# locuslab/lcp-physics

Hardware: NVIDIA H100
Metric: LCP solves/sec (LCPFunction fwd+bwd, batch=4096 x 64 contacts, fp32) (higher is better)
Workload: dtype f32 I/O and iterates; the condensed n x n KKT matrix is formed, factored and solved in f64

## Files before the change

lcp_physics_b200/csrc/lcp_cond_kernels.cu:

```cuda
#include "lcp_cond_launch.h"

namespace lcpb200 {
namespace cnd {

template <>
cudaError_t launch_cond_forward_t<LCP_T, LCP_NS>(const CFwdArgs<LCP_T>& a, int grid, cudaStream_t st) {
  if (a.prof) cond_forward_kernel<LCP_T, LCP_NS, true><<<grid, NT, a.P.smem_bytes, st>>>(a);
  else cond_forward_kernel<LCP_T, LCP_NS, false><<<grid, NT, a.P.smem_bytes, st>>>(a);
  return cudaGetLastError();
}

template <>
cudaError_t launch_cond_backward_t<LCP_T, LCP_NS>(const CBwdArgs<LCP_T>& a, int grid, cudaStream_t st) {
  if (a.prof) cond_backward_kernel<LCP_T, LCP_NS, true><<<grid, NT, a.P.smem_bytes, st>>>(a);
  else cond_backward_kernel<LCP_T, LCP_NS, false><<<grid, NT, a.P.smem_bytes, st>>>(a);
  return cudaGetLastError();
}

template <>
cudaError_t launch_cond_jvp_t<LCP_T, LCP_NS>(const CJvpArgs<LCP_T>& a, int grid, cudaStream_t st) {
  const bool dense = a.soa.mass == nullptr;
  if (a.prof) {
    if (dense) cond_jvp_kernel<LCP_T, LCP_NS, true, true><<<grid, NT, a.P.smem_bytes, st>>>(a);
    else cond_jvp_kernel<LCP_T, LCP_NS, true, false><<<grid, NT, a.P.smem_bytes, st>>>(a);
// ... 2 lines not shown
    else cond_jvp_kernel<LCP_T, LCP_NS, false, false><<<grid, NT, a.P.smem_bytes, st>>>(a);
  }
  return cudaGetLastError();
}

template <>
cudaError_t configure_cond_t<LCP_T, LCP_NS>(int smem_bytes, int dyn_max, int* occ) {
  cudaError_t e;
  const void* fns[4] = {(const void*)cond_forward_kernel<LCP_T, LCP_NS, false>, (const void*)cond_backward_kernel<LCP_T, LCP_NS, false>,
                        (const void*)cond_forward_kernel<LCP_T, LCP_NS, true>, (const void*)cond_backward_kernel<LCP_T, LCP_NS, true>};
  for (const void* f : fns)
    if ((e = cudaFuncSetAttribute(f, cudaFuncAttributeMaxDynamicSharedMemorySize, dyn_max)) != cudaSuccess) return e;
  const void* jvp[4] = {(const void*)cond_jvp_kernel<LCP_T, LCP_NS, false, false>, (const void*)cond_jvp_kernel<LCP_T, LCP_NS, true, false>,
                        (const void*)cond_jvp_kernel<LCP_T, LCP_NS, false, true>, (const void*)cond_jvp_kernel<LCP_T, LCP_NS, true, true>};
  for (const void* f : jvp)
    if ((e = cudaFuncSetAttribute(f, cudaFuncAttributeMaxDynamicSharedMemorySize, dyn_max)) != cudaSuccess) return e;
  int of = 0, ob = 0;
  if ((e = cudaOccupancyMaxActiveBlocksPerMultiprocessor(&of, fns[0], NT, smem_bytes)) != cudaSuccess) return e;
  if ((e = cudaOccupancyMaxActiveBlocksPerMultiprocessor(&ob, fns[1], NT, smem_bytes)) != cudaSuccess) return e;
  *occ = of < ob ? of : ob;
  return cudaSuccess;
}

}
}
```

lcp_physics_b200/csrc/lcp_cond_launch.h:

```cpp
#pragma once
#include <cuda_runtime.h>
#include "lcp_condensed.cuh"

namespace lcpb200 {
namespace cnd {

template <typename T, int NS> cudaError_t launch_cond_forward_t(const CFwdArgs<T>& a, int grid, cudaStream_t st);
template <typename T, int NS> cudaError_t launch_cond_backward_t(const CBwdArgs<T>& a, int grid, cudaStream_t st);
template <typename T, int NS> cudaError_t launch_cond_jvp_t(const CJvpArgs<T>& a, int grid, cudaStream_t st);
template <typename T, int NS> cudaError_t configure_cond_t(int smem_bytes, int dyn_max, int* occ);

}
}
```

lcp_physics_b200/csrc/lcp_condensed.cuh:

```cuda
#pragma once
#include "lcp_device.cuh"

namespace lcpb200 {
namespace cnd {

constexpr int NT = 256;
constexpr int UC = 8;
constexpr int CSMAX = 6;
constexpr int KS = 8;
constexpr int LMAX = 16;
constexpr int LU_BW = 2;
constexpr int MISC_BAND_LU = 4;
constexpr int CFLAG_DENSE_LU = 4;
constexpr int STATUS_UNSUPPORTED = -100;

struct CPlan {
  int ok;
  int n, m, e, N, NP, NS;
  int pcap;
  int wcap;
  int smem_bytes;
  int ctas_per_sm;
  int flags;
  int sbytes;
  int o_K, o_W, o_scr, o_bx, o_rdiag, o_Fd, o_Gd, o_As, o_x, o_rx, o_dx, o_qd, o_y, o_ry, o_dy,
      o_s, o_z, o_d, o_rz, o_ds, o_dz, o_rs2, o_red, o_rows, o_posof, o_clist, o_ccols, o_ncols, o_clcnt, o_misc;
};

__host__ __device__ inline size_t al16(size_t x) { return (x + 15) & ~(size_t)15; }
__host__ __device__ inline size_t scratch_bytes(int n, int m, int tsize) {
  return al16((size_t)2 * KS * m * 2) + al16((size_t)2 * KS * m * tsize) + al16((size_t)5 * m * 4) +
         al16((size_t)CSMAX * m * 2) + al16((size_t)8 * m * 4) + al16((size_t)LMAX * n * 2) + al16((size_t)n * 4) + 64;
}

inline size_t carve_plan(CPlan& P, int tsize) {
  size_t o = 0;
  const int n = P.n, m = P.m, e = P.e, NP = P.NP, pcap = P.pcap, wcap = P.wcap;
#define CND_TAKE(field, bytes) do { P.field = (int)o; o += al16((size_t)(bytes)); } while (0)
  size_t kb = (size_t)NP * NP * 8;
  if (scratch_bytes(n, m, tsize) > kb) kb = scratch_bytes(n, m, tsize);
  if ((size_t)8 * NP * 8 > kb) kb = (size_t)8 * NP * 8;
  { const size_t qn = (NP + 31) / 32, sl = (size_t)(NP / qn) * qn * qn * 32 * 8; if (sl > kb) kb = sl; }
  CND_TAKE(o_K, kb);
  CND_TAKE(o_W, (size_t)wcap * 8);
  CND_TAKE(o_scr, (size_t)pcap * 8);
  CND_TAKE(o_bx, (size_t)NP * 8);
  CND_TAKE(o_rdiag, (size_t)NP * 8);
  CND_TAKE(o_Fd, (size_t)wcap * tsize);
  CND_TAKE(o_Gd, (size_t)UC * pcap * tsize);
  CND_TAKE(o_As, (size_t)e * n * tsize);
  CND_TAKE(o_x, n * tsize); CND_TAKE(o_rx, n * tsize); CND_TAKE(o_dx, n * tsize); CND_TAKE(o_qd, n * tsize);
  CND_TAKE(o_y, e * tsize); CND_TAKE(o_ry, e * tsize); CND_TAKE(o_dy, e * tsize);
  CND_TAKE(o_s, m * tsize); CND_TAKE(o_z, m * tsize); CND_TAKE(o_d, m * tsize); CND_TAKE(o_rz, m * tsize);
  CND_TAKE(o_ds, m * tsize); CND_TAKE(o_dz, m * tsize); CND_TAKE(o_rs2, m * tsize);
  CND_TAKE(o_red, 192 * tsize);
  CND_TAKE(o_rows, pcap * 2);
  CND_TAKE(o_posof, m * 2);
  CND_TAKE(o_clist, LMAX * n * 2);
  CND_TAKE(o_ccols, UC * pcap);
  CND_TAKE(o_ncols, pcap);
  CND_TAKE(o_clcnt, n);
  CND_TAKE(o_misc, 16 * 4);
#undef CND_TAKE
  P.sbytes = 16 + (P.o_x - P.o_Fd) + (P.o_y - P.o_qd) + (P.o_misc - P.o_rows);
  return o;
}

extern __shared__ __align__(16) unsigned char cnd_smem[];

template <typename T>
struct CSmem {
  const CPlan& P;
  __device__ __forceinline__ explicit CSmem(const CPlan& p) : P(p) {}
#define CND_ACC(name, type) __device__ __forceinline__ type* name() const { return reinterpret_cast<type*>(cnd_smem + P.o_##name); }
  CND_ACC(K, double) CND_ACC(W, double) CND_ACC(scr, double) CND_ACC(bx, double) CND_ACC(rdiag, double)
  CND_ACC(Fd, T) CND_ACC(Gd, T) CND_ACC(As, T)
  CND_ACC(x, T) CND_ACC(rx, T) CND_ACC(dx, T) CND_ACC(qd, T) CND_ACC(y, T) CND_ACC(ry, T) CND_ACC(dy, T)
  CND_ACC(s, T) CND_ACC(z, T) CND_ACC(d, T) CND_ACC(rz, T) CND_ACC(ds, T) CND_ACC(dz, T) CND_ACC(rs2, T)
  CND_ACC(red, T)
  CND_ACC(rows, unsigned short) CND_ACC(posof, unsigned short) CND_ACC(clist, unsigned short)
  CND_ACC(ccols, unsigned char) CND_ACC(ncols, unsigned char) CND_ACC(clcnt, unsigned char)
  CND_ACC(misc, int)
#undef CND_ACC
};

struct Struct {
  int ncomp, cs;
  int sh;
  int m;
// ... 73 lines not shown
        const unsigned mask = __ballot_sync(FULL, nz);
        const int pos = c + __popc(mask & ((1u << lane) - 1u));
        if (nz && pos < KS) { vals[pos * rows + r] = v[q]; idx[pos * rows + r] = (unsigned short)(j0 + q * 32 + lane); }
        c += __popc(mask);
      }
    }
    if (c > KS) bad = 1;
    if (lane == 0) cnt[r] = c;
  }
  return bad;
}

__device__ __forceinline__ void prefetch_l2(const void* p, size_t bytes) {
  const char* c = reinterpret_cast<const char*>(p);
  for (size_t o = (size_t)threadIdx.x * 128; o < bytes; o += (size_t)NT * 128)
    asm volatile("prefetch.global.L2 [%0];" ::"l"(c + o));
}

template <typename T>
__device__ __noinline__ bool build_structure(const CPlan& P, CSmem<T>& S, Struct& st, const T* __restrict__ Q,
                                             const T* __restrict__ G, const T* __restrict__ A,
                                             const T* __restrict__ F, int* singular) {
  const int n = P.n, m = P.m, e = P.e, tid = threadIdx.x, lane = tid & 31, warp = tid >> 5, pcap = P.pcap;
  prefetch_l2(F, (size_t)m * m * sizeof(T));
  prefetch_l2(G, (size_t)m * n * sizeof(T));
  prefetch_l2(Q, (size_t)n * n * sizeof(T));
  char* sb = reinterpret_cast<char*>(S.K());
  unsigned short* Fi = reinterpret_cast<unsigned short*>(sb);
  unsigned short* Gi = Fi + (size_t)KS * m;
  size_t o = al16((size_t)2 * KS * m * 2);
  T* Fv = reinterpret_cast<T*>(sb + o);
  T* Gv = Fv + (size_t)KS * m;
  o += al16((size_t)2 * KS * m * sizeof(T));
  int* Fcnt = reinterpret_cast<int*>(sb + o);
  int* Gcnt = Fcnt + m;
  int* label = Gcnt + m;
  int* cidx = label + m;
  int* memcnt = cidx + m;
  o += al16((size_t)5 * m * 4);
  unsigned short* memb = reinterpret_cast<unsigned short*>(sb + o);
  o += al16((size_t)CSMAX * m * 2);
  unsigned* cmap = reinterpret_cast<unsigned*>(sb + o);
  o += al16((size_t)8 * m * 4);
  unsigned short* cl_tmp = reinterpret_cast<unsigned short*>(sb + o);
  o += al16((size_t)LMAX * n * 2);
  int* cl_cnt = reinterpret_cast<int*>(sb + o);
  int* flags = S.misc();

  if (tid < 16) flags[tid] = 0;
// ... 729 lines not shown
  const T NEG_INF = -INFINITY, POS_INF = INFINITY;
  T mx[2] = {NEG_INF, NEG_INF};
  T mn[2] = {POS_INF, POS_INF};
  T any[2] = {T(0), T(0)};
  for (int i = threadIdx.x; i < m; i += NT) {
    const T az = -z[i] / dz[i], as = -s[i] / ds[i];
    mx[0] = nan_max(mx[0], az);
    mx[1] = nan_max(mx[1], as);
    if (dz[i] > T(0)) any[0] = T(1); else mn[0] = nan_min(mn[0], az);
    if (ds[i] > T(0)) any[1] = T(1); else mn[1] = nan_min(mn[1], as);
  }
  T v[6] = {mx[0], mx[1], -mn[0], -mn[1], any[0], any[1]};
  block_reduce<T, 6>(v, OpMax(), NEG_INF, red);
  const T fz = (v[0] > T(1)) ? v[0] : T(1);
  const T fs = (v[1] > T(1)) ? v[1] : T(1);
  step_z = (v[4] > T(0)) ? nan_min(-v[2], fz) : -v[2];
  step_s = (v[5] > T(0)) ? nan_min(-v[3], fs) : -v[3];
}

template <typename T>
struct CFwdArgs {
  CPlan P;
  int B;
  const T *Q, *p, *G, *h, *A, *b, *F;
  T *zhat, *nu, *lam, *slack, *resid;
  int *status, *iters;
  T eps;
  int not_improved_lim, max_iter;
  long long* prof;
  EngineSoA<T> soa;
  unsigned char* ssave;
};

template <typename T>
struct CBwdArgs {
  CPlan P;
  int B;
  int R, chunks;
  const T *Q, *G, *A, *F;
  const T *zhat, *nu, *lam, *slack, *g;
  T *dQ, *dp, *dG, *dh, *dA, *db, *dF;
  int* done;
  const int* only;
  unsigned flags;
  const unsigned char* sload;
  EngineSoA<T> soa;
  T *dmass, *dinertia, *dv, *dfext, *dnormal, *dp1, *dp2, *dmu, *drest;
  long long* prof;
};

__device__ __forceinline__ void copy16(unsigned char* dst, const unsigned char* src, int bytes) {
  const uint4* s4 = reinterpret_cast<const uint4*>(src);
  uint4* d4 = reinterpret_cast<uint4*>(dst);
  for (int i = threadIdx.x; i < (bytes >> 4); i += NT) d4[i] = s4[i];
}

__device__ __forceinline__ void save_structure(const CPlan& P, const Struct& st, bool ok, unsigned char* dst) {
  if (threadIdx.x == 0) *reinterpret_cast<int4*>(dst) = make_int4(ok ? st.ncomp : -1, st.cs, st.sh, st.m);
  if (!ok) return;
  const int c1 = P.o_x - P.o_Fd, c2 = P.o_y - P.o_qd, c3 = P.o_misc - P.o_rows;
  copy16(dst + 16, cnd_smem + P.o_Fd, c1);
  copy16(dst + 16 + c1, cnd_smem + P.o_qd, c2);
  copy16(dst + 16 + c1 + c2, cnd_smem + P.o_rows, c3);
}

__device__ __forceinline__ bool load_structure(const CPlan& P, Struct& st, const unsigned char* src) {
  const int4 hd = *reinterpret_cast<const int4*>(src);
  st.ncomp = hd.x; st.cs = hd.y; st.sh = hd.z; st.m = hd.w;
  if (hd.x < 0) return false;
  const int c1 = P.o_x - P.o_Fd, c2 = P.o_y - P.o_qd, c3 = P.o_misc - P.o_rows;
  copy16(cnd_smem + P.o_Fd, src + 16, c1);
  copy16(cnd_smem + P.o_qd, src + 16 + c1, c2);
  copy16(cnd_smem + P.o_rows, src + 16 + c1 + c2, c3);
  return true;
}

template <typename T>
struct SzResid { T sz, resid; };

template <typename T, int CS>
__device__ __noinline__ SzResid<T> fwd_residuals(const CFwdArgs<T>& a, CSmem<T> S, Struct st, int sc) {
  const int nc_ = st.ncomp;
  const CPlan& P = a.P;
  const int n = P.n, m = st.m, e = P.e, tid = threadIdx.x, pcap = P.pcap;
  const T* p = a.p + (size_t)sc * n;
  const T* h = a.h + (size_t)sc * P.m;
  const T* b = e > 0 ? a.b + (size_t)sc * e : nullptr;
  for (int c = tid; c < n; c += NT) {
    T acc = 0;
    const int cnt = S.clcnt()[c];
    for (int l = 0; l < cnt; ++l) {
      const int cp = S.clist()[l * n + c], cc = cp >> 3, pp = cp & 7;
#pragma unroll
      for (int r = 0; r < CS; ++r) {
        const int i = S.rows()[r * nc_ + cc];
        if (i != 0xFFFF) acc = fma(S.Gd()[(size_t)pp * pcap + r * nc_ + cc], S.z()[i], acc);
      }
// ... 138 lines not shown
    pf.lap(CPH_STEP);
    solve_kkt<T, CS, NS>(P, S, st, pf, nullptr, S.rs2(), nullptr, nullptr, S.rx(), S.rz(), S.rs2(), S.ry());
    fwd_step<T>(P, S, m);
    pf.lap(CPH_STEP);
    pf.count(CPH_FACTORS);
    pf.count(CPH_SOLVES, 2);
  }
  if (threadIdx.x == 0) { a.status[sc] = status; a.iters[sc] = it; if (a.resid) a.resid[sc] = best; }
}

template <typename T, int NS, bool PROF>
__global__ void __launch_bounds__(NT, (NS <= 6) ? 2 : 1) cond_forward_kernel(const __grid_constant__ CFwdArgs<T> a) {
  const CPlan& P = a.P;
  CSmem<T> S(P);
  const int n = P.n, m = P.m, e = P.e, tid = threadIdx.x;
  __shared__ int singular_s;
  const T NANV = nan("");
  Prof<PROF> pf(PROF ? a.prof + (size_t)blockIdx.x * CPH_COUNT : nullptr);
  for (int sc = blockIdx.x; sc < a.B; sc += gridDim.x) {
    if (tid == 0) singular_s = 0;
    __syncthreads();
    pf.start();
    Struct st;
    const bool ok = a.soa.mass
        ? build_structure_soa<T>(P, S, st, a.soa, sc, e > 0 ? a.A + (size_t)sc * e * n : nullptr, &singular_s)
        : build_structure<T>(P, S, st, a.Q + (size_t)sc * n * n, a.G + (size_t)sc * m * n,
                             e > 0 ? a.A + (size_t)sc * e * n : nullptr, a.F + (size_t)sc * m * m, &singular_s);
    __syncthreads();
    if (a.ssave) save_structure(P, st, ok, a.ssave + (size_t)sc * P.sbytes);
    pf.lap(CPH_STRUCT);
    if (!ok) {
      if (singular_s) {
        for (int i = tid; i < n; i += NT) a.zhat[(size_t)sc * n + i] = NANV;
        for (int i = tid; i < m; i += NT) { a.lam[(size_t)sc * m + i] = NANV; a.slack[(size_t)sc * m + i] = NANV; }
        for (int i = tid; i < e; i += NT) a.nu[(size_t)sc * e + i] = NANV;
        if (tid == 0) { a.status[sc] = -1; a.iters[sc] = 0; if (a.resid) a.resid[sc] = NANV; }
      } else if (tid == 0) {
        a.status[sc] = STATUS_UNSUPPORTED;
        a.iters[sc] = 0;
      }
      __syncthreads();
      continue;
    }
    if constexpr (LU_BW < NS - 1) mark_band_lu<T>(P, S, st);
    switch (st.cs) {
      case 1: forward_scene<T, NS, 1>(a, S, st, pf, sc); break;
      case 2: forward_scene<T, NS, 2>(a, S, st, pf, sc); break;
      case 3: forward_scene<T, NS, 3>(a, S, st, pf, sc); break;
      case 4: forward_scene<T, NS, 4>(a, S, st, pf, sc); break;
      case 5: forward_scene<T, NS, 5>(a, S, st, pf, sc); break;
      default: forward_scene<T, NS, 6>(a, S, st, pf, sc); break;
    }
    __syncthreads();
  }
}
// ... 481 lines not shown
```

lcp_physics_b200/csrc/lcpb200.cu:

```cuda
#include <cuda_runtime.h>
#include <stdio.h>
#include <string.h>
#include <algorithm>
#include <cfloat>
#include <climits>
#include <cmath>
#include <new>
#include <string>
#include <type_traits>
#include <vector>

#include "../../include/lcpb200.h"
#include "lcp_assemble.cuh"
#include "lcp_launch.h"
#include "lcp_cond_launch.h"
#include "lcp_band_launch.h"
#include "lcp_contacts.cuh"
#include "lcp_ray_launch.h"

using namespace lcpb200;
using cnd::CPlan;

static thread_local std::string g_err;
static int fail(const std::string& s) { g_err = s; return 1; }
// ... 18 lines not shown
};

struct DevBuf {
  void* p = nullptr;
  size_t bytes = 0;
  cudaError_t ensure(size_t need) {
    if (need <= bytes) return cudaSuccess;
    if (p) cudaFree(p);
    p = nullptr; bytes = 0;
    cudaError_t e = cudaMalloc(&p, need);
    if (e == cudaSuccess) bytes = need;
    return e;
  }
  void release() { if (p) cudaFree(p); p = nullptr; bytes = 0; }
};

struct lcpb200_handle_s {
  int dtype, n, m, e, device;
  int num_sms, smem_optin;
  Plan plan;
  int max_grid;
  CPlan cplan;
  int cond_grid = 0;
  static const int NSLOT = 2;
  void* ws = nullptr;
  size_t ws_bytes = 0;
  int ws_ctas = 0;
  DevBuf d_flag[NSLOT];
  DevBuf d_ph;
  bool dual_ok = true;
  bnd::BPlan bplan;
  int bplan_mode = -1;
  DevBuf d_bwsd, d_bwsi;
  int bws_ctas = 0;
  cudaStream_t streams[NSLOT] = {nullptr, nullptr};
  DevBuf d_in[7], d_out[6], d_bwd[16];
  long long* prof = nullptr;
  long long* cprof = nullptr;
  DevBuf d_struct;
  int struct_B = 0;
  DevBuf d_R;
  int retained_B = 0;
  bool retained_R = false;
};

static int pad_ld(int cols, int elem_bytes) {
  const int wpe = elem_bytes / 4;
  int ld = cols;
  while ((ld * wpe) % 32 != 4 || (ld * elem_bytes) % 16 != 0) ++ld;
  return ld;
}

template <typename T>
static int make_plan(lcpb200_handle_s* h) {
  Plan& P = h->plan;
  const int n = h->n, m = h->m, e = h->e;
  constexpr int NB = Blk<T>::NB, VC = VecOf<T>::VC;
  const int w = (int)sizeof(T);
  memset(&P, 0, sizeof(P));
  P.n = n; P.m = m; P.e = e;
  P.mp = ((m + NB - 1) / NB) * NB;
  const int mp = P.mp;
  P.nt = (mp >= 96 || n >= 96) ? 512 : (mp >= 64 ? 256 : 128);
// ... 85 lines not shown
  C.pcap = (m + 7) & ~7;
  C.flags = getenv("LCPB200_COND_FLAGS") ? atoi(getenv("LCPB200_COND_FLAGS")) : 3;
  const int dyn_max = h->smem_optin - 1024;
  const int target = NS <= 6 ? 2 : 1;
  const int per_cta_target = (228 * 1024) / target - 1024 - 64;
  int best = -1;
  for (int want = target; want >= 1 && best < 0; --want) {
    const int lim = std::min(dyn_max, want == target ? per_cta_target : (228 * 1024) / want - 1024 - 64);
    for (int mult = cnd::CSMAX; mult >= 1; --mult) {
      C.wcap = mult * C.pcap;
      const size_t bytes = cnd::carve_plan(C, (int)sizeof(T));
      if ((long long)bytes <= lim) { best = (int)bytes; break; }
      if (mult <= 4) break;
    }
  }
  if (best < 0) return 0;
  C.smem_bytes = best;
  int occ = 0;
#define CALL_CFG(NSV) cnd::configure_cond_t<T, NSV>(C.smem_bytes, dyn_max, &occ)
  const cudaError_t ce = LCPB200_NS_DISPATCH(NS, CALL_CFG);
#undef CALL_CFG
  if (ce != cudaSuccess) return fail(std::string("condensed kernel configuration: ") + cudaGetErrorString(ce));
  if (occ < 1) return 0;
  C.ctas_per_sm = occ;
  h->cond_grid = occ * h->num_sms;
  C.ok = 1;
  return 0;
}

extern "C" int lcpb200_version(void) { return LCPB200_VERSION; }
extern "C" const char* lcpb200_last_error_string(void) { return g_err.c_str(); }

extern "C" int lcpb200_create(int dtype, int n, int m, int e, int device, lcpb200_handle_t* out) {
  if (!out) return fail("out == NULL");
  *out = nullptr;
  if (dtype != LCPB200_F32 && dtype != LCPB200_F64) return fail("dtype must be LCPB200_F32 or LCPB200_F64");
  if (n <= 0 || m <= 0 || e < 0) return fail("need n > 0, m > 0, e >= 0");
  DeviceGuard dg_;
  CK(dg_.set(device));
  lcpb200_handle_s* h = new (std::nothrow) lcpb200_handle_s();
  if (!h) return fail("out of host memory");
  h->dtype = dtype; h->n = n; h->m = m; h->e = e; h->device = device;
  cudaError_t ce;
  if ((ce = cudaDeviceGetAttribute(&h->num_sms, cudaDevAttrMultiProcessorCount, device)) != cudaSuccess ||
      (ce = cudaDeviceGetAttribute(&h->smem_optin, cudaDevAttrMaxSharedMemoryPerBlockOptin, device)) != cudaSuccess) {
    delete h;
// ... 12 lines not shown
  memset(&h->bplan, 0, sizeof(h->bplan));
  *out = h;
  return 0;
}

static int ensure_ws(lcpb200_handle_s* h, int B) {
  const int ctas = std::min(B, h->max_grid);
  if (ctas <= h->ws_ctas) return 0;
  const size_t esz = h->dtype == LCPB200_F32 ? 4 : 8;
  const size_t need = (size_t)h->plan.ws_per_cta * esz * (size_t)ctas * lcpb200_handle_s::NSLOT;
  if (h->ws) { CK(cudaDeviceSynchronize()); CK(cudaFree(h->ws)); h->ws = nullptr; h->ws_bytes = 0; h->ws_ctas = 0; }
  CK(cudaMalloc(&h->ws, need));
  h->ws_bytes = need;
  h->ws_ctas = ctas;
  return 0;
}

extern "C" int lcpb200_destroy(lcpb200_handle_t h) {
  if (!h) return 0;
  DeviceGuard dg_;
  dg_.set(h->device);
  if (h->ws) cudaFree(h->ws);
  h->d_struct.release();
  if (h->prof) cudaFree(h->prof);
  if (h->cprof) cudaFree(h->cprof);
  for (auto& s : h->streams) if (s) cudaStreamDestroy(s);
  for (auto& b : h->d_in) b.release();
  for (auto& b : h->d_out) b.release();
  for (auto& b : h->d_bwd) b.release();
  for (auto& b : h->d_flag) b.release();
  h->d_ph.release();
  h->d_bwsd.release();
  h->d_bwsi.release();
  h->d_R.release();
  delete h;
  return 0;
}

extern "C" size_t lcpb200_workspace_bytes(lcpb200_handle_t h) { return h ? h->ws_bytes : 0; }

extern "C" int lcpb200_describe(lcpb200_handle_t h, char* buf, size_t len) {
  if (!h || !buf) return fail("null argument");
  const Plan& P = h->plan;
  static const char* modes[3] = {"smem", "smem-split(U12 in L2)", "L2"};
  const CPlan& C = h->cplan;
  char cbuf[256];
  if (C.ok)
    snprintf(cbuf, sizeof(cbuf), "condensed KKT: N=%d(pad %d) fp64 LU in registers, threads=%d smem=%dB CTAs/SM=%d grid<=%d "
             "(forward%s; unstructured scenes fall back to dual)", C.N, C.NP, cnd::NT, C.smem_bytes, C.ctas_per_sm,
             h->cond_grid, h->dtype == LCPB200_F32 ? "+backward" : "");
  else
    snprintf(cbuf, sizeof(cbuf), "condensed KKT: n/a");
  snprintf(buf, len,
           "dtype=%s n=%d m=%d(pad %d) e=%d | %s | dual: threads=%d smem=%dB T:%s m1=%d ldT=%d ldL=%d G:%s Qinv:%s grid<=%d "
           "ws/CTA=%lldB sms=%d",
           h->dtype == LCPB200_F32 ? "f32" : "f64", P.n, P.m, P.mp, P.e, cbuf, P.nt, P.smem_bytes, modes[P.mode], P.m1,
           P.ldT, P.ldL, P.G_smem ? "smem" : "L2", P.Qi_smem ? "smem" : "L2", h->max_grid,
           (long long)(P.ws_per_cta * (h->dtype == LCPB200_F32 ? 4 : 8)), h->num_sms);
  return 0;
}

template <typename T>
static int launch_forward(lcpb200_handle_s* h, int slot, int B, const void* Q, const void* p, const void* G,
                          const void* hv, const void* A, const void* b, const void* F, double eps,
                          int not_improved_lim, int max_iter, void* zhat, void* nu, void* lam, void* slack,
                          int32_t* status, int32_t* iters, void* resid, void* Rsave, cudaStream_t st,
                          unsigned char* ssave = nullptr) {
  const bool cond = h->cplan.ok != 0;
  if (cond) {
    cnd::CFwdArgs<T> c;
    c.P = h->cplan;
    c.B = B;
    c.Q = (const T*)Q; c.p = (const T*)p; c.G = (const T*)G; c.h = (const T*)hv;
    c.A = (const T*)A; c.b = (const T*)b; c.F = (const T*)F;
    c.zhat = (T*)zhat; c.nu = (T*)nu; c.lam = (T*)lam; c.slack = (T*)slack; c.resid = (T*)resid;
    c.status = status; c.iters = iters;
    c.eps = (T)eps; c.not_improved_lim = not_improved_lim; c.max_iter = max_iter;
    memset(&c.soa, 0, sizeof(c.soa));
    c.ssave = ssave;
    c.prof = h->cprof ? h->cprof + (size_t)slot * h->cond_grid * cnd::CPH_COUNT : nullptr;
    const int cgrid = std::min(B, h->cond_grid);
#define CALL_FWD(NSV) cnd::launch_cond_forward_t<T, NSV>(c, cgrid, st)
    const cudaError_t ce = LCPB200_NS_DISPATCH(h->cplan.NS, CALL_FWD);
#undef CALL_FWD
    CK(ce);
    Rsave = nullptr;
  }
  if (int rc = ensure_ws(h, B)) return rc;
  FwdArgs<T> a;
  a.P = h->plan;
  a.B = B;
  a.Q = (const T*)Q; a.p = (const T*)p; a.G = (const T*)G; a.h = (const T*)hv;
  a.A = (const T*)A; a.b = (const T*)b; a.F = (const T*)F;
  a.zhat = (T*)zhat; a.nu = (T*)nu; a.lam = (T*)lam; a.slack = (T*)slack; a.resid = (T*)resid;
  a.status = status; a.iters = iters;
  a.eps = (T)eps; a.not_improved_lim = not_improved_lim; a.max_iter = max_iter;
  a.Rsave = (T*)Rsave;
  a.fallback_only = cond ? 1 : 0;
  a.ws = (T*)h->ws + (size_t)slot * h->plan.ws_per_cta * h->ws_ctas;
  a.prof = h->prof ? h->prof + (size_t)slot * h->max_grid * PH_COUNT : nullptr;
  const int grid = std::min(B, h->ws_ctas);
  const int mode = h->plan.mode;
// ... 119 lines not shown
                          const void* A, const void* b, const void* F, const void* zhat, const void* nu,
                          const void* lam, const void* slack, const void* status, const void* iters,
                          int max_iter) {
  if (!h) return fail("null handle");
  if (B < 0) return fail("B < 0");
  if (!Q || !p || !G || !hv || !F) return fail("Q, p, G, h, F must be non-NULL");
  if (h->e > 0 && (!A || !b)) return fail("handle was created with e > 0 but A or b is NULL");
  if (!zhat || !lam || !slack || !status || !iters) return fail("zhat, lam, slack, status, iters must be non-NULL");
  if (h->e > 0 && !nu) return fail("nu must be non-NULL when e > 0");
  if (max_iter < 0) return fail("max_iter < 0");
  return 0;
}

extern "C" int lcpb200_forward(lcpb200_handle_t h, int B, const void* Q, const void* p, const void* G,
                               const void* hv, const void* A, const void* b, const void* F, double eps,
                               int not_improved_lim, int max_iter, void* zhat, void* nu, void* lam, void* slack,
                               int32_t* status, int32_t* iters, void* resid, void* Rsave, void* stream) {
  if (int rc = check_fwd_args(h, B, Q, p, G, hv, A, b, F, zhat, nu, lam, slack, status, iters, max_iter)) return rc;
  if (!h->dual_ok) return fail("this handle serves the engine entry points only (problem too large for the dense API)");
  if (B == 0) return 0;
  DeviceGuard dg_;
  CK(dg_.set(h->device));
  cudaStream_t st = (cudaStream_t)stream;
  unsigned char* ssave = nullptr;
  h->struct_B = 0;
  if (h->cplan.ok) {
    if ((size_t)B * h->cplan.sbytes > h->d_struct.bytes) CK(cudaDeviceSynchronize());
    CK(h->d_struct.ensure((size_t)B * h->cplan.sbytes));
    ssave = (unsigned char*)h->d_struct.p;
  }
  const int rc = h->dtype == LCPB200_F32
             ? launch_forward<float>(h, 0, B, Q, p, G, hv, A, b, F, eps, not_improved_lim, max_iter, zhat, nu, lam,
                                     slack, status, iters, resid, Rsave, st, ssave)
             : launch_forward<double>(h, 0, B, Q, p, G, hv, A, b, F, eps, not_improved_lim, max_iter, zhat, nu, lam,
                                      slack, status, iters, resid, Rsave, st, ssave);
  if (rc == 0 && ssave) h->struct_B = B;
  return rc;
}

static int check_dense_derivative(lcpb200_handle_t h, int R, int B, const void* Q, const void* G, const void* F,
                                  const void* A, const void* zhat, const void* nu, const void* lam, const void* slack) {
  if (!h) return fail("null handle");
  if (!h->dual_ok) return fail("this handle serves the engine entry points only (problem too large for the dense API)");
  if (R < 1) return fail("need R >= 1");
  if (B < 0) return fail("B < 0");
  if ((long long)R * B > INT_MAX) return fail("R * B exceeds INT_MAX");
  if (!Q || !G || !F || !zhat || !lam || !slack) return fail("Q, G, F, zhat, lam, slack must be non-NULL");
  if (h->e > 0 && (!A || !nu)) return fail("A and nu must be non-NULL when e > 0");
  return 0;
}

static const unsigned char* saved_structure(const lcpb200_handle_s* h, int B, unsigned flags) {
  return ((flags & LCPB200_BWD_REUSE_STRUCTURE) && h->cplan.ok && h->struct_B == B) ? (const unsigned char*)h->d_struct.p
                                                                                      : nullptr;
}

extern "C" int lcpb200_backward_batched(lcpb200_handle_t h, int R, int B, const void* Q, const void* G, const void* A,
                                        const void* F, const void* zhat, const void* nu, const void* lam,
                                        const void* slack, const void* g, void* dQ, void* dp, void* dG, void* dh,
// ... 91 lines not shown
extern "C" int lcpb200_forward_host(lcpb200_handle_t h, int B, const void* Q, const void* p, const void* G,
                                    const void* hv, const void* A, const void* b, const void* F, double eps,
                                    int not_improved_lim, int max_iter, void* zhat, void* nu, void* lam,
                                    void* slack, int32_t* status, int32_t* iters, void* resid) {
  if (int rc = check_fwd_args(h, B, Q, p, G, hv, A, b, F, zhat, nu, lam, slack, status, iters, max_iter)) return rc;
  if (!h->dual_ok) return fail("this handle serves the engine entry points only (problem too large for the dense API)");
  if (B == 0) return 0;
  DeviceGuard dg_;
  CK(dg_.set(h->device));
  if (int rc = ensure_streams(h)) return rc;
  const size_t w = h->dtype == LCPB200_F32 ? 4 : 8;
  const size_t n = h->n, m = h->m, e = h->e;
  const size_t in_sz[7] = {n * n * w, n * w, m * n * w, m * w, e * n * w, e * w, m * m * w};
  const void* in_src[7] = {Q, p, G, hv, A, b, F};
  const size_t out_sz[6] = {n * w, e * w, m * w, m * w, 4, 4};
  void* out_dst[6] = {zhat, nu, lam, slack, status, iters};
  for (int i = 0; i < 7; ++i) if (in_sz[i]) CK(h->d_in[i].ensure(in_sz[i] * B));
  for (int i = 0; i < 6; ++i) if (out_sz[i]) CK(h->d_out[i].ensure(out_sz[i] * B));
  DevBuf& d_resid = h->d_bwd[15];
  if (resid) CK(d_resid.ensure(w * B));
  h->retained_B = 0;
  const bool keepR = !h->cplan.ok && (m * m * w * (size_t)B) <= ((size_t)8 << 30);
  if (keepR) CK(h->d_R.ensure(m * m * w * (size_t)B));
  const int C = chunk_scenes(h, B);
  int k = 0;
  for (int s0 = 0; s0 < B; s0 += C, ++k) {
    const int cb = std::min(C, B - s0);
    const int slot = k % lcpb200_handle_s::NSLOT;
    cudaStream_t st = h->streams[slot];
    for (int i = 0; i < 7; ++i)
      if (in_sz[i] && in_src[i])
        CK(cudaMemcpyAsync((char*)h->d_in[i].p + in_sz[i] * s0, (const char*)in_src[i] + in_sz[i] * s0,
                           in_sz[i] * cb, cudaMemcpyHostToDevice, st));
    auto at = [&](DevBuf& bf, size_t per) -> void* { return per ? (char*)bf.p + per * s0 : nullptr; };
    int rc = h->dtype == LCPB200_F32
                 ? launch_forward<float>(h, slot, cb, at(h->d_in[0], in_sz[0]), at(h->d_in[1], in_sz[1]),
                                         at(h->d_in[2], in_sz[2]), at(h->d_in[3], in_sz[3]), at(h->d_in[4], in_sz[4]),
                                         at(h->d_in[5], in_sz[5]), at(h->d_in[6], in_sz[6]), eps, not_improved_lim,
                                         max_iter, at(h->d_out[0], out_sz[0]), at(h->d_out[1], out_sz[1]),
                                         at(h->d_out[2], out_sz[2]), at(h->d_out[3], out_sz[3]),
                                         (int32_t*)at(h->d_out[4], 4), (int32_t*)at(h->d_out[5], 4),
                                         resid ? (char*)d_resid.p + w * s0 : nullptr,
                                         keepR ? (char*)h->d_R.p + m * m * w * s0 : nullptr, st)
                 : launch_forward<double>(h, slot, cb, at(h->d_in[0], in_sz[0]), at(h->d_in[1], in_sz[1]),
                                          at(h->d_in[2], in_sz[2]), at(h->d_in[3], in_sz[3]), at(h->d_in[4], in_sz[4]),
                                          at(h->d_in[5], in_sz[5]), at(h->d_in[6], in_sz[6]), eps, not_improved_lim,
                                          max_iter, at(h->d_out[0], out_sz[0]), at(h->d_out[1], out_sz[1]),
                                          at(h->d_out[2], out_sz[2]), at(h->d_out[3], out_sz[3]),
                                          (int32_t*)at(h->d_out[4], 4), (int32_t*)at(h->d_out[5], 4),
                                          resid ? (char*)d_resid.p + w * s0 : nullptr,
                                          keepR ? (char*)h->d_R.p + m * m * w * s0 : nullptr, st);
    if (rc) return rc;
    for (int i = 0; i < 6; ++i)
      if (out_sz[i] && out_dst[i])
        CK(cudaMemcpyAsync((char*)out_dst[i] + out_sz[i] * s0, (char*)h->d_out[i].p + out_sz[i] * s0,
                           out_sz[i] * cb, cudaMemcpyDeviceToHost, st));
    if (resid)
      CK(cudaMemcpyAsync((char*)resid + w * s0, (char*)d_resid.p + w * s0, w * cb, cudaMemcpyDeviceToHost, st));
  }
  for (auto& s : h->streams) CK(cudaStreamSynchronize(s));
  h->retained_B = B;
  h->retained_R = keepR;
  return 0;
}

extern "C" int lcpb200_backward_host(lcpb200_handle_t h, int B, const void* Q, const void* G, const void* A,
                                     const void* F, const void* zhat, const void* nu, const void* lam,
                                     const void* slack, const void* g, void* dQ, void* dp, void* dG, void* dh,
                                     void* dA, void* db, void* dF, unsigned flags) {
  if (!h) return fail("null handle");
  if (!h->dual_ok) return fail("this handle serves the engine entry points only (problem too large for the dense API)");
  if (B < 0) return fail("B < 0");
  const bool retained = (Q == nullptr);
  if (retained) {
// ... 103 lines not shown
  }
  return 0;
}

static int check_engine(lcpb200_handle_t h, int B, int nb, int nc, int mode) {
  if (!h) return fail("null handle");
  if (B < 0 || nb <= 0 || nc <= 0) return fail("need B >= 0, nb > 0, nc > 0");
  if (mode != 0 && mode != 1) return fail("mode must be 0 (solve_dynamics) or 1 (post_stabilization)");
  if (!h->cplan.ok && h->dtype != LCPB200_F64)
    return fail("engine entry points: n + e > 128 needs the large-scene kernel, which is fp64 only");
  if (h->n != 3 * nb || h->m != (mode == 0 ? 4 : 1) * nc)
    return fail("handle was created for other sizes: need n = 3 nb and m = 4 nc (mode 0) or nc (mode 1)");
  return 0;
}

template <typename T>
static int engine_forward_t(lcpb200_handle_s* h, int B, const EngineIn& in, const void* A, const void* b, double eps,
                            int not_improved_lim, int max_iter, void* zhat, void* nu, void* lam, void* slack,
                            int32_t* status, int32_t* iters, void* resid, cudaStream_t st) {
  CK(h->d_ph.ensure(sizeof(T) * (size_t)B * (h->n + h->m)));
  cnd::CFwdArgs<T> c;
  c.P = h->cplan;
  c.B = B;
  c.Q = nullptr; c.G = nullptr; c.F = nullptr;
  c.A = (const T*)A; c.b = (const T*)b;
  fill_soa<T>(c.soa, in, B, h->n, (T*)h->d_ph.p);
  c.ssave = nullptr;
  c.p = c.soa.p_s; c.h = c.soa.h_s;
  c.zhat = (T*)zhat; c.nu = (T*)nu; c.lam = (T*)lam; c.slack = (T*)slack; c.resid = (T*)resid;
  c.status = status; c.iters = iters;
  c.eps = (T)eps; c.not_improved_lim = not_improved_lim; c.max_iter = max_iter;
  c.prof = h->cprof;
  const int cgrid = std::min(B, h->cond_grid);
#define CALL_FWD(NSV) cnd::launch_cond_forward_t<T, NSV>(c, cgrid, st)
  const cudaError_t ce = LCPB200_NS_DISPATCH(h->cplan.NS, CALL_FWD);
#undef CALL_FWD
  CK(ce);
  return 0;
}

extern "C" int lcpb200_engine_forward(lcpb200_handle_t h, int B, int nb, int nc, int mode, double dt,
                                      const void* mass, const void* inertia, const void* v, const void* fext,
                                      const void* normal, const void* p1, const void* p2, const int32_t* body1,
                                      const int32_t* body2, const int32_t* contact_count, const void* mu,
                                      const void* restitution, const void* A, const void* b, double eps, int not_improved_lim, int max_iter, void* zhat,
                                      void* nu, void* lam, void* slack, int32_t* status, int32_t* iters, void* resid,
                                      void* stream) {
  if (int rc = check_engine(h, B, nb, nc, mode)) return rc;
  if (!mass || !inertia || !v || !normal || !p1 || !p2 || !body1 || !body2 || !restitution) return fail("engine_forward: NULL input");
  if (mode == 0 && (!fext || !mu)) return fail("engine_forward: fext and mu are needed for mode 0");
// ... 429 lines not shown
```

Baseline: 331,500.

## Split structure discovery into a separate low-smem scan kernel before the condensed solve

Moves sparsity-structure discovery (build_structure) out of the condensed forward kernel into its own kernel. The new kernel uses a slimmer shared-memory plan, skips the L2 prefetch, and writes a structure blob that the forward kernel then loads. The aim is to run the memory-heavy scan at higher occupancy than the big-smem solver and to keep the solver kernel free of the dense Q/G/F reads. In exchange it adds a kernel launch and a global round trip for the structure blob, and the solver no longer gets the prefetch overlap.

```diff
diff --git a/lcp_physics_b200/csrc/lcp_cond_kernels.cu b/lcp_physics_b200/csrc/lcp_cond_kernels.cu
--- a/lcp_physics_b200/csrc/lcp_cond_kernels.cu
+++ b/lcp_physics_b200/csrc/lcp_cond_kernels.cu
@@ -48,5 +48,21 @@
   return cudaSuccess;
 }
 
+#if LCP_NS == 2
+template <>
+cudaError_t launch_cond_structure_t<LCP_T>(const CScanArgs<LCP_T>& a, int grid, cudaStream_t st) {
+  cond_structure_kernel<LCP_T><<<grid, NT, a.P.smem_bytes, st>>>(a);
+  return cudaGetLastError();
+}
+
+template <>
+cudaError_t configure_cond_structure_t<LCP_T>(int smem_bytes, int dyn_max, int* occ) {
+  const void* f = (const void*)cond_structure_kernel<LCP_T>;
+  cudaError_t e = cudaFuncSetAttribute(f, cudaFuncAttributeMaxDynamicSharedMemorySize, dyn_max);
+  if (e != cudaSuccess) return e;
+  return cudaOccupancyMaxActiveBlocksPerMultiprocessor(occ, f, NT, smem_bytes);
+}
+#endif
+
 }
 }
diff --git a/lcp_physics_b200/csrc/lcp_cond_launch.h b/lcp_physics_b200/csrc/lcp_cond_launch.h
--- a/lcp_physics_b200/csrc/lcp_cond_launch.h
+++ b/lcp_physics_b200/csrc/lcp_cond_launch.h
@@ -9,6 +9,8 @@
 template <typename T, int NS> cudaError_t launch_cond_backward_t(const CBwdArgs<T>& a, int grid, cudaStream_t st);
 template <typename T, int NS> cudaError_t launch_cond_jvp_t(const CJvpArgs<T>& a, int grid, cudaStream_t st);
 template <typename T, int NS> cudaError_t configure_cond_t(int smem_bytes, int dyn_max, int* occ);
+template <typename T> cudaError_t launch_cond_structure_t(const CScanArgs<T>& a, int grid, cudaStream_t st);
+template <typename T> cudaError_t configure_cond_structure_t(int smem_bytes, int dyn_max, int* occ);
 
 }
 }
diff --git a/lcp_physics_b200/csrc/lcp_condensed.cuh b/lcp_physics_b200/csrc/lcp_condensed.cuh
--- a/lcp_physics_b200/csrc/lcp_condensed.cuh
+++ b/lcp_physics_b200/csrc/lcp_condensed.cuh
@@ -12,6 +12,7 @@
 constexpr int LU_BW = 2;
 constexpr int MISC_BAND_LU = 4;
 constexpr int CFLAG_DENSE_LU = 4;
+constexpr int CFLAG_NO_L2_PREFETCH = 8;
 constexpr int STATUS_UNSUPPORTED = -100;
 
 struct CPlan {
@@ -23,6 +24,7 @@
   int ctas_per_sm;
   int flags;
   int sbytes;
+  int sseg[3];
   int o_K, o_W, o_scr, o_bx, o_rdiag, o_Fd, o_Gd, o_As, o_x, o_rx, o_dx, o_qd, o_y, o_ry, o_dy,
       o_s, o_z, o_d, o_rz, o_ds, o_dz, o_rs2, o_red, o_rows, o_posof, o_clist, o_ccols, o_ncols, o_clcnt, o_misc;
 };
@@ -33,10 +35,32 @@
          al16((size_t)CSMAX * m * 2) + al16((size_t)8 * m * 4) + al16((size_t)LMAX * n * 2) + al16((size_t)n * 4) + 64;
 }
 
+#define CND_TAKE(field, bytes) do { P.field = (int)o; o += al16((size_t)(bytes)); } while (0)
+inline size_t carve_segment(CPlan& P, int tsize, int seg, size_t o) {
+  const size_t o0 = o;
+  const int n = P.n, m = P.m, e = P.e, pcap = P.pcap;
+  if (seg == 0) {
+    CND_TAKE(o_Fd, (size_t)P.wcap * tsize);
+    CND_TAKE(o_Gd, (size_t)UC * pcap * tsize);
+    CND_TAKE(o_As, (size_t)e * n * tsize);
+  } else if (seg == 1) {
+    CND_TAKE(o_qd, n * tsize);
+  } else {
+    CND_TAKE(o_rows, pcap * 2);
+    CND_TAKE(o_posof, m * 2);
+    CND_TAKE(o_clist, LMAX * n * 2);
+    CND_TAKE(o_ccols, UC * pcap);
+    CND_TAKE(o_ncols, pcap);
+    CND_TAKE(o_clcnt, n);
+  }
+  P.sseg[seg] = (int)(o - o0);
+  P.sbytes = 16 + P.sseg[0] + P.sseg[1] + P.sseg[2];
+  return o;
+}
+
 inline size_t carve_plan(CPlan& P, int tsize) {
   size_t o = 0;
   const int n = P.n, m = P.m, e = P.e, NP = P.NP, pcap = P.pcap, wcap = P.wcap;
-#define CND_TAKE(field, bytes) do { P.field = (int)o; o += al16((size_t)(bytes)); } while (0)
   size_t kb = (size_t)NP * NP * 8;
   if (scratch_bytes(n, m, tsize) > kb) kb = scratch_bytes(n, m, tsize);
   if ((size_t)8 * NP * 8 > kb) kb = (size_t)8 * NP * 8;
@@ -46,25 +70,32 @@
   CND_TAKE(o_scr, (size_t)pcap * 8);
   CND_TAKE(o_bx, (size_t)NP * 8);
   CND_TAKE(o_rdiag, (size_t)NP * 8);
-  CND_TAKE(o_Fd, (size_t)wcap * tsize);
-  CND_TAKE(o_Gd, (size_t)UC * pcap * tsize);
-  CND_TAKE(o_As, (size_t)e * n * tsize);
-  CND_TAKE(o_x, n * tsize); CND_TAKE(o_rx, n * tsize); CND_TAKE(o_dx, n * tsize); CND_TAKE(o_qd, n * tsize);
+  o = carve_segment(P, tsize, 0, o);
+  CND_TAKE(o_x, n * tsize); CND_TAKE(o_rx, n * tsize); CND_TAKE(o_dx, n * tsize);
+  o = carve_segment(P, tsize, 1, o);
   CND_TAKE(o_y, e * tsize); CND_TAKE(o_ry, e * tsize); CND_TAKE(o_dy, e * tsize);
   CND_TAKE(o_s, m * tsize); CND_TAKE(o_z, m * tsize); CND_TAKE(o_d, m * tsize); CND_TAKE(o_rz, m * tsize);
   CND_TAKE(o_ds, m * tsize); CND_TAKE(o_dz, m * tsize); CND_TAKE(o_rs2, m * tsize);
   CND_TAKE(o_red, 192 * tsize);
-  CND_TAKE(o_rows, pcap * 2);
-  CND_TAKE(o_posof, m * 2);
-  CND_TAKE(o_clist, LMAX * n * 2);
-  CND_TAKE(o_ccols, UC * pcap);
-  CND_TAKE(o_ncols, pcap);
-  CND_TAKE(o_clcnt, n);
+  o = carve_segment(P, tsize, 2, o);
   CND_TAKE(o_misc, 16 * 4);
+  return o;
+}
+
+inline CPlan carve_scan_plan(const CPlan& solver, int tsize) {
+  CPlan P = solver;
+  P.o_W = P.o_scr = P.o_bx = P.o_rdiag = P.o_x = P.o_rx = P.o_dx = P.o_y = P.o_ry = P.o_dy = 0;
+  P.o_s = P.o_z = P.o_d = P.o_rz = P.o_ds = P.o_dz = P.o_rs2 = P.o_red = 0;
+  P.flags |= CFLAG_NO_L2_PREFETCH;
+  size_t o = 0;
+  CND_TAKE(o_K, scratch_bytes(P.n, P.m, tsize));
+  for (int seg = 0; seg < 3; ++seg) o = carve_segment(P, tsize, seg, o);
+  CND_TAKE(o_misc, 16 * 4);
+  P.smem_bytes = (int)o;
+  P.ctas_per_sm = 0;
+  return P;
+}
 #undef CND_TAKE
-  P.sbytes = 16 + (P.o_x - P.o_Fd) + (P.o_y - P.o_qd) + (P.o_misc - P.o_rows);
-  return o;
-}
 
 extern __shared__ __align__(16) unsigned char cnd_smem[];
 
@@ -184,9 +215,11 @@
                                              const T* __restrict__ G, const T* __restrict__ A,
                                              const T* __restrict__ F, int* singular) {
   const int n = P.n, m = P.m, e = P.e, tid = threadIdx.x, lane = tid & 31, warp = tid >> 5, pcap = P.pcap;
-  prefetch_l2(F, (size_t)m * m * sizeof(T));
-  prefetch_l2(G, (size_t)m * n * sizeof(T));
-  prefetch_l2(Q, (size_t)n * n * sizeof(T));
+  if (!(P.flags & CFLAG_NO_L2_PREFETCH)) {
+    prefetch_l2(F, (size_t)m * m * sizeof(T));
+    prefetch_l2(G, (size_t)m * n * sizeof(T));
+    prefetch_l2(Q, (size_t)n * n * sizeof(T));
+  }
   char* sb = reinterpret_cast<char*>(S.K());
   unsigned short* Fi = reinterpret_cast<unsigned short*>(sb);
   unsigned short* Gi = Fi + (size_t)KS * m;
@@ -962,14 +995,22 @@
 struct CFwdArgs {
   CPlan P;
   int B;
-  const T *Q, *p, *G, *h, *A, *b, *F;
+  const T *p, *h, *A, *b;
   T *zhat, *nu, *lam, *slack, *resid;
   int *status, *iters;
   T eps;
   int not_improved_lim, max_iter;
   long long* prof;
   EngineSoA<T> soa;
-  unsigned char* ssave;
+  const unsigned char* sload;
+};
+
+template <typename T>
+struct CScanArgs {
+  CPlan P;
+  int B;
+  const T *Q, *G, *A, *F;
+  unsigned char* out;
 };
 
 template <typename T>
@@ -989,30 +1030,56 @@
   long long* prof;
 };
 
+constexpr int SBLOB_UNSUPPORTED = -1;
+constexpr int SBLOB_SINGULAR_Q = -2;
+
 __device__ __forceinline__ void copy16(unsigned char* dst, const unsigned char* src, int bytes) {
   const uint4* s4 = reinterpret_cast<const uint4*>(src);
   uint4* d4 = reinterpret_cast<uint4*>(dst);
   for (int i = threadIdx.x; i < (bytes >> 4); i += NT) d4[i] = s4[i];
 }
 
-__device__ __forceinline__ void save_structure(const CPlan& P, const Struct& st, bool ok, unsigned char* dst) {
-  if (threadIdx.x == 0) *reinterpret_cast<int4*>(dst) = make_int4(ok ? st.ncomp : -1, st.cs, st.sh, st.m);
+__device__ __forceinline__ void save_structure(const CPlan& P, const Struct& st, bool ok, bool singular,
+                                               unsigned char* dst) {
+  if (threadIdx.x == 0)
+    *reinterpret_cast<int4*>(dst) = make_int4(ok ? st.ncomp : (singular ? SBLOB_SINGULAR_Q : SBLOB_UNSUPPORTED),
+                                              ok ? st.cs : 0, ok ? st.sh : 0, ok ? st.m : 0);
   if (!ok) return;
-  const int c1 = P.o_x - P.o_Fd, c2 = P.o_y - P.o_qd, c3 = P.o_misc - P.o_rows;
+  const int c1 = P.sseg[0], c2 = P.sseg[1], c3 = P.sseg[2];
   copy16(dst + 16, cnd_smem + P.o_Fd, c1);
   copy16(dst + 16 + c1, cnd_smem + P.o_qd, c2);
   copy16(dst + 16 + c1 + c2, cnd_smem + P.o_rows, c3);
 }
 
-__device__ __forceinline__ bool load_structure(const CPlan& P, Struct& st, const unsigned char* src) {
+__device__ __forceinline__ bool load_structure(const CPlan& P, Struct& st, const unsigned char* src,
+                                               int* singular = nullptr) {
   const int4 hd = *reinterpret_cast<const int4*>(src);
   st.ncomp = hd.x; st.cs = hd.y; st.sh = hd.z; st.m = hd.w;
+  if (singular) *singular = hd.x == SBLOB_SINGULAR_Q;
   if (hd.x < 0) return false;
-  const int c1 = P.o_x - P.o_Fd, c2 = P.o_y - P.o_qd, c3 = P.o_misc - P.o_rows;
+  const int c1 = P.sseg[0], c2 = P.sseg[1], c3 = P.sseg[2];
   copy16(cnd_smem + P.o_Fd, src + 16, c1);
   copy16(cnd_smem + P.o_qd, src + 16 + c1, c2);
   copy16(cnd_smem + P.o_rows, src + 16 + c1 + c2, c3);
   return true;
+}
+
+template <typename T>
+__global__ void __launch_bounds__(NT, 3) cond_structure_kernel(const __grid_constant__ CScanArgs<T> a) {
+  const CPlan& P = a.P;
+  CSmem<T> S(P);
+  const int n = P.n, m = P.m, e = P.e, tid = threadIdx.x;
+  __shared__ int singular_s;
+  for (int sc = blockIdx.x; sc < a.B; sc += gridDim.x) {
+    if (tid == 0) singular_s = 0;
+    __syncthreads();
+    Struct st;
+    const bool ok = build_structure<T>(P, S, st, a.Q + (size_t)sc * n * n, a.G + (size_t)sc * m * n,
+                                       e > 0 ? a.A + (size_t)sc * e * n : nullptr, a.F + (size_t)sc * m * m, &singular_s);
+    __syncthreads();
+    save_structure(P, st, ok, singular_s != 0, a.out + (size_t)sc * P.sbytes);
+    __syncthreads();
+  }
 }
 
 template <typename T>
@@ -1197,15 +1264,14 @@
     __syncthreads();
     pf.start();
     Struct st;
+    int singular = 0;
     const bool ok = a.soa.mass
         ? build_structure_soa<T>(P, S, st, a.soa, sc, e > 0 ? a.A + (size_t)sc * e * n : nullptr, &singular_s)
-        : build_structure<T>(P, S, st, a.Q + (size_t)sc * n * n, a.G + (size_t)sc * m * n,
-                             e > 0 ? a.A + (size_t)sc * e * n : nullptr, a.F + (size_t)sc * m * m, &singular_s);
-    __syncthreads();
-    if (a.ssave) save_structure(P, st, ok, a.ssave + (size_t)sc * P.sbytes);
+        : load_structure(P, st, a.sload + (size_t)sc * P.sbytes, &singular);
+    __syncthreads();
     pf.lap(CPH_STRUCT);
     if (!ok) {
-      if (singular_s) {
+      if (singular || singular_s) {
         for (int i = tid; i < n; i += NT) a.zhat[(size_t)sc * n + i] = NANV;
         for (int i = tid; i < m; i += NT) { a.lam[(size_t)sc * m + i] = NANV; a.slack[(size_t)sc * m + i] = NANV; }
         for (int i = tid; i < e; i += NT) a.nu[(size_t)sc * e + i] = NANV;
diff --git a/lcp_physics_b200/csrc/lcpb200.cu b/lcp_physics_b200/csrc/lcpb200.cu
--- a/lcp_physics_b200/csrc/lcpb200.cu
+++ b/lcp_physics_b200/csrc/lcpb200.cu
@@ -64,6 +64,8 @@
   int max_grid;
   CPlan cplan;
   int cond_grid = 0;
+  CPlan splan;
+  int scan_grid = 0;
   static const int NSLOT = 2;
   void* ws = nullptr;
   size_t ws_bytes = 0;
@@ -81,6 +83,7 @@
   long long* cprof = nullptr;
   DevBuf d_struct;
   int struct_B = 0;
+  DevBuf d_hstruct;
   DevBuf d_R;
   int retained_B = 0;
   bool retained_R = false;
@@ -212,6 +215,15 @@
 #undef CALL_CFG
   if (ce != cudaSuccess) return fail(std::string("condensed kernel configuration: ") + cudaGetErrorString(ce));
   if (occ < 1) return 0;
+  CPlan S = cnd::carve_scan_plan(C, (int)sizeof(T));
+  int socc = 0;
+  const cudaError_t se = cnd::configure_cond_structure_t<T>(S.smem_bytes, dyn_max, &socc);
+  if (se != cudaSuccess) return fail(std::string("structure scan configuration: ") + cudaGetErrorString(se));
+  if (socc < 1) return 0;
+  S.ctas_per_sm = socc;
+  S.ok = 1;
+  h->splan = S;
+  h->scan_grid = socc * h->num_sms;
   C.ctas_per_sm = occ;
   h->cond_grid = occ * h->num_sms;
   C.ok = 1;
@@ -270,6 +282,7 @@
   dg_.set(h->device);
   if (h->ws) cudaFree(h->ws);
   h->d_struct.release();
+  h->d_hstruct.release();
   if (h->prof) cudaFree(h->prof);
   if (h->cprof) cudaFree(h->cprof);
   for (auto& s : h->streams) if (s) cudaStreamDestroy(s);
@@ -292,11 +305,12 @@
   const Plan& P = h->plan;
   static const char* modes[3] = {"smem", "smem-split(U12 in L2)", "L2"};
   const CPlan& C = h->cplan;
-  char cbuf[256];
+  char cbuf[320];
   if (C.ok)
     snprintf(cbuf, sizeof(cbuf), "condensed KKT: N=%d(pad %d) fp64 LU in registers, threads=%d smem=%dB CTAs/SM=%d grid<=%d "
-             "(forward%s; unstructured scenes fall back to dual)", C.N, C.NP, cnd::NT, C.smem_bytes, C.ctas_per_sm,
-             h->cond_grid, h->dtype == LCPB200_F32 ? "+backward" : "");
+             "(forward%s; unstructured scenes fall back to dual); structure scan: smem=%dB CTAs/SM=%d grid<=%d",
+             C.N, C.NP, cnd::NT, C.smem_bytes, C.ctas_per_sm, h->cond_grid, h->dtype == LCPB200_F32 ? "+backward" : "",
+             h->splan.smem_bytes, h->splan.ctas_per_sm, h->scan_grid);
   else
     snprintf(cbuf, sizeof(cbuf), "condensed KKT: n/a");
   snprintf(buf, len,
@@ -313,19 +327,25 @@
                           const void* hv, const void* A, const void* b, const void* F, double eps,
                           int not_improved_lim, int max_iter, void* zhat, void* nu, void* lam, void* slack,
                           int32_t* status, int32_t* iters, void* resid, void* Rsave, cudaStream_t st,
-                          unsigned char* ssave = nullptr) {
+                          unsigned char* sbuf) {
   const bool cond = h->cplan.ok != 0;
   if (cond) {
+    if (!sbuf) return fail("launch_forward: no structure buffer");
+    cnd::CScanArgs<T> s;
+    s.P = h->splan;
+    s.B = B;
+    s.Q = (const T*)Q; s.G = (const T*)G; s.A = (const T*)A; s.F = (const T*)F;
+    s.out = sbuf;
+    CK(cnd::launch_cond_structure_t<T>(s, std::min(B, h->scan_grid), st));
     cnd::CFwdArgs<T> c;
     c.P = h->cplan;
     c.B = B;
-    c.Q = (const T*)Q; c.p = (const T*)p; c.G = (const T*)G; c.h = (const T*)hv;
-    c.A = (const T*)A; c.b = (const T*)b; c.F = (const T*)F;
+    c.p = (const T*)p; c.h = (const T*)hv; c.A = (const T*)A; c.b = (const T*)b;
     c.zhat = (T*)zhat; c.nu = (T*)nu; c.lam = (T*)lam; c.slack = (T*)slack; c.resid = (T*)resid;
     c.status = status; c.iters = iters;
     c.eps = (T)eps; c.not_improved_lim = not_improved_lim; c.max_iter = max_iter;
     memset(&c.soa, 0, sizeof(c.soa));
-    c.ssave = ssave;
+    c.sload = sbuf;
     c.prof = h->cprof ? h->cprof + (size_t)slot * h->cond_grid * cnd::CPH_COUNT : nullptr;
     const int cgrid = std::min(B, h->cond_grid);
 #define CALL_FWD(NSV) cnd::launch_cond_forward_t<T, NSV>(c, cgrid, st)
@@ -491,19 +511,19 @@
   DeviceGuard dg_;
   CK(dg_.set(h->device));
   cudaStream_t st = (cudaStream_t)stream;
-  unsigned char* ssave = nullptr;
+  unsigned char* sbuf = nullptr;
   h->struct_B = 0;
   if (h->cplan.ok) {
     if ((size_t)B * h->cplan.sbytes > h->d_struct.bytes) CK(cudaDeviceSynchronize());
     CK(h->d_struct.ensure((size_t)B * h->cplan.sbytes));
-    ssave = (unsigned char*)h->d_struct.p;
+    sbuf = (unsigned char*)h->d_struct.p;
   }
   const int rc = h->dtype == LCPB200_F32
              ? launch_forward<float>(h, 0, B, Q, p, G, hv, A, b, F, eps, not_improved_lim, max_iter, zhat, nu, lam,
-                                     slack, status, iters, resid, Rsave, st, ssave)
+                                     slack, status, iters, resid, Rsave, st, sbuf)
              : launch_forward<double>(h, 0, B, Q, p, G, hv, A, b, F, eps, not_improved_lim, max_iter, zhat, nu, lam,
-                                      slack, status, iters, resid, Rsave, st, ssave);
-  if (rc == 0 && ssave) h->struct_B = B;
+                                      slack, status, iters, resid, Rsave, st, sbuf);
+  if (rc == 0 && sbuf) h->struct_B = B;
   return rc;
 }
 
@@ -641,6 +661,8 @@
   h->retained_B = 0;
   const bool keepR = !h->cplan.ok && (m * m * w * (size_t)B) <= ((size_t)8 << 30);
   if (keepR) CK(h->d_R.ensure(m * m * w * (size_t)B));
+  const size_t sb = h->cplan.ok ? (size_t)h->cplan.sbytes : 0;
+  if (sb) CK(h->d_hstruct.ensure(sb * B));
   const int C = chunk_scenes(h, B);
   int k = 0;
   for (int s0 = 0; s0 < B; s0 += C, ++k) {
@@ -660,7 +682,8 @@
                                          at(h->d_out[2], out_sz[2]), at(h->d_out[3], out_sz[3]),
                                          (int32_t*)at(h->d_out[4], 4), (int32_t*)at(h->d_out[5], 4),
                                          resid ? (char*)d_resid.p + w * s0 : nullptr,
-                                         keepR ? (char*)h->d_R.p + m * m * w * s0 : nullptr, st)
+                                         keepR ? (char*)h->d_R.p + m * m * w * s0 : nullptr, st,
+                                         sb ? (unsigned char*)h->d_hstruct.p + sb * s0 : nullptr)
                  : launch_forward<double>(h, slot, cb, at(h->d_in[0], in_sz[0]), at(h->d_in[1], in_sz[1]),
                                           at(h->d_in[2], in_sz[2]), at(h->d_in[3], in_sz[3]), at(h->d_in[4], in_sz[4]),
                                           at(h->d_in[5], in_sz[5]), at(h->d_in[6], in_sz[6]), eps, not_improved_lim,
@@ -668,7 +691,8 @@
                                           at(h->d_out[2], out_sz[2]), at(h->d_out[3], out_sz[3]),
                                           (int32_t*)at(h->d_out[4], 4), (int32_t*)at(h->d_out[5], 4),
                                           resid ? (char*)d_resid.p + w * s0 : nullptr,
-                                          keepR ? (char*)h->d_R.p + m * m * w * s0 : nullptr, st);
+                                          keepR ? (char*)h->d_R.p + m * m * w * s0 : nullptr, st,
+                                          sb ? (unsigned char*)h->d_hstruct.p + sb * s0 : nullptr);
     if (rc) return rc;
     for (int i = 0; i < 6; ++i)
       if (out_sz[i] && out_dst[i])
@@ -818,10 +842,9 @@
   cnd::CFwdArgs<T> c;
   c.P = h->cplan;
   c.B = B;
-  c.Q = nullptr; c.G = nullptr; c.F = nullptr;
   c.A = (const T*)A; c.b = (const T*)b;
   fill_soa<T>(c.soa, in, B, h->n, (T*)h->d_ph.p);
-  c.ssave = nullptr;
+  c.sload = nullptr;
   c.p = c.soa.p_s; c.h = c.soa.h_s;
   c.zhat = (T*)zhat; c.nu = (T*)nu; c.lam = (T*)lam; c.slack = (T*)slack; c.resid = (T*)resid;
   c.status = status; c.iters = iters;
```

Measured after the change: 336,900, median of 6. 1.6% higher.
